# zoj613/OccuSpytial

Measured on AMD Instinct MI355X. Metric: Gibbs iterations/sec on 100x100 ICAR lattice, 4 chains; 1/2/4/8 GPUs, higher is better.
Workload: dtype f64; 1 GPU; 100x100 queen ICAR lattice, 10000 sites, 5 visits/site, p=q=2, 4 chains per GPU batched in every kernel (BASELINE configs[1] data, the metric's 4 chains); chains_per_gpu=4, total_chains=4, sites=10000, visit_rows=50000, parallelism=chains sharded 4/GPU, no data-path collective; one GPU, communicator=single process, problem_transport=none, krylov_cap=0, stalls=0, solve_form=k_iter, one XCD per chain, solve_workgroups_per_chain=23, main_stream_cus=160, fused_fallbacks=0, threads_per_block=64

## Files before the change

### occuspytial_amd/csrc/occ_kernels.hpp

```cpp
#pragma once
#include <float.h>
#include <hip/hip_runtime.h>
#include <stdint.h>

#include "occ_plan.hpp"
#include "occ_rng.hpp"
#include "occ_state.hpp"

namespace occ {


#ifndef OCC_SLOT_ALIGN
#define OCC_SLOT_ALIGN 8
#endif
struct alignas(OCC_SLOT_ALIGN) Slot {
    double beta1, beta, oldb, alfa, dbar, epsln, phibar, rhs1, rhs2, tnorm2, gmax, gmin, cs, sn, root;
    double ibeta;
    int itn;
    int istop;
    int done;
    int pad;
};

#define OCC_SLOT_FIELDS(X) \
// ... 279 lines not shown

__device__ __forceinline__ void reduce_partials_lds(const double *part, int nq, int nw, double *lds_out)
{
    const int lane = threadIdx.x & 63, wave = threadIdx.x >> 6, nwb = blockDim.x >> 6;
    for (int qi = wave; qi < nq; qi += nwb) {
        double s = 0.0;
        const double *pq = part + (size_t)qi * nw;
        for (int b0 = lane; b0 < nw; b0 += 512) {
            double v[8];
#pragma unroll
            for (int r = 0; r < 8; ++r) {
                const int b = b0 + 64 * r;
                const double t = pq[min(b, nw - 1)];
                v[r] = (b < nw) ? t : 0.0;
            }
#pragma unroll
            for (int r = 0; r < 8; ++r) s += v[r];
        }
        s = wave_sum(s);
        if (lane == 0) lds_out[qi] = s;
    }
    __syncthreads();
}

struct PartialEmitter {
    double *out;
    int nb, blk, nq;
    __device__ __forceinline__ void emit(int t, double v)
    {
        extern __shared__ double s_gpart[];
        const double r = wave_sum(v);
        if ((threadIdx.x & 63) == 0) {
            if (blockDim.x == 64) out[(size_t)t * nb + blk] = r;
            else s_gpart[(threadIdx.x >> 6) * nq + t] = r;
        }
    }
    __device__ __forceinline__ void finish()
    {
        extern __shared__ double s_gpart[];
        if (blockDim.x == 64) return;
        __syncthreads();
        const int nw = blockDim.x >> 6;
        for (int t = threadIdx.x; t < nq; t += blockDim.x) {
            double acc = 0.0;
            for (int w = 0; w < nw; ++w) acc += s_gpart[w * nq + t];
            out[(size_t)t * nb + blk] = acc;
        }
    }
};
__host__ __device__ constexpr size_t generic_lds_bytes(int nq, int threads) { return threads == 64 ? 0 : sizeof(double) * (size_t)(threads / 64) * nq; }

__device__ __forceinline__ void slice_of(const Ctx &c, int i, int &base, int &width)
{
    const int slice = i >> 6;
    if (c.ell_w > 0) {
        width = c.ell_w;
        base = slice * c.ell_w * 64;
    } else {
        base = c.sell_ptr[slice];
        width = (c.sell_ptr[slice + 1] - base) >> 6;
    }
}




__device__ __forceinline__ double eta_rhs_site(double om, double xb, double z, double en, double up, double sqrt_tau)
{
    const double b = fma(-om, xb, z - 0.5);
    return fma(sqrt_tau, up, fma(sqrt(om), en, b));
}
__device__ __forceinline__ double eta_project(double2 xz, double a) { return fma(a, xz.y, xz.x); }
__device__ __forceinline__ double beta_rhs_term(double om, double eta, double z) { return fma(-om, eta, z - 0.5); }

__device__ inline bool precision_mvnorm_dev(int d, const double *acc ,
                                            const double *prec0, const double *pbm, uint64_t key, uint32_t it,
                                            uint32_t stream, double *U, double *work, double *out, const double *eps_inj = nullptr)
{
    double *r = work, *o = work + d;
    int t = 0;
    for (int a = 0; a < d; ++a)
        for (int b = a; b < d; ++b) U[a * d + b] = acc[t++] + prec0[a * d + b];
    for (int a = 0; a < d; ++a) r[a] = acc[t++] + pbm[a];
    bool ok = true;
    for (int j = 0; j < d; ++j) {
        double s = U[j * d + j];
        for (int k = 0; k < j; ++k) s -= U[k * d + j] * U[k * d + j];
        if (!(s > 0.0)) ok = false;
        const double ujj = sqrt(s);
        U[j * d + j] = ujj;
        for (int i = j + 1; i < d; ++i) {
            double v = U[j * d + i];
            for (int k = 0; k < j; ++k) v -= U[k * d + j] * U[k * d + i];
            U[j * d + i] = v / ujj;
        }
    }
    for (int i = d - 1; i >= 0; --i) {
        o[i] = 0.0;
    }
    for (int k = 0; k < d; ++k) {
        const double e = eps_inj ? eps_inj[k] : block_normal(key, (uint32_t)k, 0, it, stream);
        for (int i = k; i < d; ++i) o[i] += U[k * d + i] * e;
    }
    for (int i = 0; i < d; ++i) o[i] += r[i];
    for (int i = 0; i < d; ++i) {
        double v = o[i];
        for (int k = 0; k < i; ++k) v -= U[k * d + i] * o[k];
        o[i] = v / U[i * d + i];
    }
    for (int i = d - 1; i >= 0; --i) {
        double v = o[i];
        for (int k = i + 1; k < d; ++k) v -= U[i * d + k] * o[k];
        o[i] = v / U[i * d + i];
    }
    for (int i = 0; i < d; ++i) out[i] = o[i];
    return ok;
}

template <int D, class Normal>
__device__ __forceinline__ bool precision_mvnorm_with(const double (&acc)[nacc(D)], const double *prec0, const double *pbm, double (&out)[D],
                                                      Normal normal)
{
    double U[D][D], r[D], o[D];
    int t = 0;
#pragma unroll
    for (int a = 0; a < D; ++a)
#pragma unroll
        for (int b = a; b < D; ++b) U[a][b] = acc[t++] + prec0[a * D + b];
#pragma unroll
    for (int a = 0; a < D; ++a) r[a] = acc[t++] + pbm[a];
    bool ok = true;
#pragma unroll
    for (int j = 0; j < D; ++j) {
        double sj = U[j][j];
#pragma unroll
        for (int k = 0; k < j; ++k) sj -= U[k][j] * U[k][j];
        if (!(sj > 0.0)) ok = false;
        const double ujj = sqrt(sj);
        U[j][j] = ujj;
#pragma unroll
        for (int i = j + 1; i < D; ++i) {
            double v = U[j][i];
#pragma unroll
            for (int k = 0; k < j; ++k) v -= U[k][j] * U[k][i];
            U[j][i] = v / ujj;
        }
    }
#pragma unroll
    for (int i = 0; i < D; ++i) o[i] = 0.0;
#pragma unroll
    for (int k = 0; k < D; ++k) {
        const double e = normal(k);
#pragma unroll
        for (int i = k; i < D; ++i) o[i] += U[k][i] * e;
    }
#pragma unroll
    for (int i = 0; i < D; ++i) o[i] += r[i];
#pragma unroll
    for (int i = 0; i < D; ++i) {
        double v = o[i];
#pragma unroll
        for (int k = 0; k < i; ++k) v -= U[k][i] * o[k];
        o[i] = v / U[i][i];
    }
#pragma unroll
    for (int i = D - 1; i >= 0; --i) {
        double v = o[i];
#pragma unroll
        for (int k = i + 1; k < D; ++k) v -= U[i][k] * o[k];
        o[i] = v / U[i][i];
    }
#pragma unroll
    for (int i = 0; i < D; ++i) out[i] = o[i];
    return ok;
}

template <int D>
__device__ __forceinline__ bool precision_mvnorm_reg(const double (&acc)[nacc(D)], const double *prec0, const double *pbm,
                                                     uint64_t key, uint32_t it, uint32_t stream, double (&out)[D],
                                                     const double *eps_inj = nullptr)
{
    return precision_mvnorm_with<D>(acc, prec0, pbm, out,
                                    [=](int k) { return eps_inj ? eps_inj[k] : block_normal(key, (uint32_t)k, 0, it, stream); });
}


enum : int { SYNC_MAIN = 0, SYNC_ALPHA = 16, SYNC_NOISE = 32, SYNC_MAIN_SEQ = 48, SYNC_SIDE_SEQ = 52, SYNC_ABORT = 56, SYNC_DEBUG = 57, SYNC_WORDS = 64 };
constexpr unsigned SYNC_SPIN_LIMIT = 1u << 19;

__device__ __forceinline__ unsigned sync_read(const unsigned *p)
{
    return __hip_atomic_load(p, __ATOMIC_RELAXED, __HIP_MEMORY_SCOPE_AGENT);
}
__device__ __forceinline__ void sync_set(unsigned *p, unsigned v)
{
    __hip_atomic_store(p, v, __ATOMIC_RELAXED, __HIP_MEMORY_SCOPE_AGENT);
}
__device__ __forceinline__ bool sync_wait(unsigned *sync, int word, unsigned target)
{
    unsigned spins = 0;
    while ((int)(sync_read(sync + word) - target) < 0) {
        __builtin_amdgcn_s_sleep(4);
        ++spins;
        if ((spins & 63u) == 0u && sync_read(sync + SYNC_ABORT) != 0u) return false;
        if (spins > SYNC_SPIN_LIMIT) {
            sync_set(sync + SYNC_ABORT, 1u);
            return false;
        }
    }
    return true;
}
__device__ __forceinline__ double load_agent(const double *p)
{
    return __hip_atomic_load(p, __ATOMIC_RELAXED, __HIP_MEMORY_SCOPE_AGENT);
}
__device__ __forceinline__ uint64_t uniform_u64(uint64_t v)
{
    const unsigned lo = (unsigned)__builtin_amdgcn_readfirstlane((int)(unsigned)v), hi = (unsigned)__builtin_amdgcn_readfirstlane((int)(unsigned)(v >> 32));
    return ((uint64_t)hi << 32) | lo;
}
__device__ __forceinline__ double uniform_f64(double v) { return __longlong_as_double((long long)uniform_u64((uint64_t)__double_as_longlong(v))); }

__global__ void __launch_bounds__(64) k_stream_probe_wait(unsigned *w)
{
    if (threadIdx.x != 0) return;
    unsigned seen = 0u, spins = 0u;
    for (; spins < (1u << 13); ++spins) {
        if (sync_read(w) != 0u) { seen = 1u; break; }
        __builtin_amdgcn_s_sleep(16);
    }
    w[16] = seen;
    w[17] = spins;
}
__global__ void __launch_bounds__(64) k_stream_probe_set(unsigned *w)
{
    if (threadIdx.x == 0) sync_set(w, 1u);
}

__global__ void __launch_bounds__(256) k_checksum(const unsigned char *__restrict__ data, unsigned long long bytes, unsigned long long *__restrict__ out)
{
    const unsigned long long nw = (bytes + 7ull) / 8ull;
    unsigned long long acc = 0ull;
    for (unsigned long long i = (unsigned long long)blockIdx.x * blockDim.x + threadIdx.x; i < nw; i += (unsigned long long)gridDim.x * blockDim.x) {
        unsigned long long w = 0ull;
        if (8ull * i + 8ull <= bytes) w = *reinterpret_cast<const unsigned long long *>(data + 8ull * i);
        else
            for (unsigned long long b = 8ull * i; b < bytes; ++b) w |= (unsigned long long)data[b] << (8ull * (b - 8ull * i));
        unsigned long long x = w + 0x9E3779B97F4A7C15ull * (i + 1ull);
        x = (x ^ (x >> 30)) * 0xBF58476D1CE4E5B9ull;
        x = (x ^ (x >> 27)) * 0x94D049BB133111EBull;
        acc += x ^ (x >> 31);
    }
    atomicAdd(out, acc);
}

__global__ void __launch_bounds__(256) k_snapshot(const double *__restrict__ eta, double *__restrict__ s_eta, const uint8_t *__restrict__ z, uint8_t *__restrict__ s_z,
                                                  const double2 *__restrict__ x, double2 *__restrict__ s_x, unsigned long long count,
                                                  const double *__restrict__ theta, double *__restrict__ s_theta, unsigned long long count_theta,
                                                  unsigned long long *__restrict__ clock,
                                                  ChainScalars *__restrict__ scs, int n_chains, int parity, uint32_t n_iter, uint32_t burnin, uint32_t keep)
{
    if (clock != nullptr && blockIdx.x == 0 && threadIdx.x < 4) clock[threadIdx.x] = threadIdx.x == 0 ? ~0ull : 0ull;
    if (scs != nullptr && blockIdx.x == 0) {
        for (int ch = (int)threadIdx.x; ch < n_chains; ch += (int)blockDim.x) {
            ChainScalars &sc = scs[ch];
            Ctl &ctl = sc.ctl[parity];
            sc.it_base = ctl.it;
            sc.it_stop = ctl.it + n_iter;
            sc.burnin = burnin;
            sc.keep = keep;
            ctl.koff = 0;
        }
    }
    for (unsigned long long i = (unsigned long long)blockIdx.x * blockDim.x + threadIdx.x; i < count; i += (unsigned long long)gridDim.x * blockDim.x) {
        s_eta[i] = eta[i];
        s_z[i] = z[i];
        s_x[i] = x[i];
    }
    for (unsigned long long i = (unsigned long long)blockIdx.x * blockDim.x + threadIdx.x; i < count_theta; i += (unsigned long long)gridDim.x * blockDim.x) s_theta[i] = theta[i];
}

__global__ void __launch_bounds__(64) k_gate(const Ctx *__restrict__ cp, ChainScalars *__restrict__ scs)
{
    const Ctx &c = *cp;
    if (c.sync == nullptr || threadIdx.x != 0) return;
    const unsigned j = c.sync[SYNC_SIDE_SEQ];
    if (c.sync[SYNC_DEBUG] != 0u) return;
    sync_set(c.sync + SYNC_NOISE, j);
    if (!sync_wait(c.sync, SYNC_MAIN, j)) scs[0].err = -2;
}

#define OCC_KARGS const Ctx *__restrict__ cp, ChainScalars *__restrict__ scs, Slot *__restrict__ slots, int chain_base, int e

__device__ __forceinline__ double quad_site(const Ctx &c, const double *eta, int i, double eta_i)
{
    const int lane = i & 63;
    int base, width;
    slice_of(c, i, base, width);
    double qe = c.qdiag[i] * eta_i;
    for (int k = 0; k < width; ++k) qe = fma(c.sell_val[base + k * 64 + lane], eta[c.sell_col[base + k * 64 + lane]], qe);
    return eta_i * qe;
}

template <int P>
__device__ __forceinline__ void omega_b_body(const Ctx &c, uint64_t key, const double (&beta)[P], int chain, uint32_t it, int blk,
                                             bool per_wave = false)
{
    const int n = c.n;
    const double *eta = c.eta + (size_t)chain * n;
    double om = 0.0;
    {
        const int i = blk * blockDim.x + threadIdx.x;
        if (i < n) {
            double xb = 0.0;
#pragma unroll
            for (int a = 0; a < P; ++a) xb += c.Xt[(size_t)a * n + i] * beta[a];
            om = pg1_draw(key, (uint32_t)i, it, STREAM_OMEGA_B, xb + eta[i]);
        }
    }
    int t = (int)threadIdx.x;
    asm volatile("" : "+v"(t));
    const int i = blk * (int)blockDim.x + t;
    double quad[1] = {0.0};
    if (i < n) {
        c.omega_b[it & 1][(size_t)chain * n + i] = om;
        quad[0] = quad_site(c, eta, i, eta[i]);
    }
    if (per_wave) {
        const double t = wave_sum(quad[0]);
        const int slice = blk * (int)(blockDim.x >> 6) + (int)(threadIdx.x >> 6);
        if ((threadIdx.x & 63) == 0 && slice < c.nb_n) c.part_quad[(size_t)chain * c.nb_n + slice] = t;
        return;
    }
    block_partials<1>(quad, c.part_quad + (size_t)chain * c.nb_n, c.nb_n, blk);
}

__device__ __forceinline__ void omega_b_body_g(const Ctx &c, const ChainScalars &sc, int chain, uint32_t it, int blk, bool per_wave = false)
{
    const int n = c.n, i = blk * blockDim.x + threadIdx.x;
    double quad[1] = {0.0};
    if (i < n) {
        const size_t ci = (size_t)chain * n + i;
        const double *eta = c.eta + (size_t)chain * n;
        double xb = 0.0;
        for (int a = 0; a < c.p; ++a) xb += c.Xt[(size_t)a * n + i] * sc.beta[a];
        const double eta_i = eta[i];
        c.omega_b[it & 1][ci] = pg1_draw(sc.key, (uint32_t)i, it, STREAM_OMEGA_B, xb + eta_i);
        quad[0] = quad_site(c, eta, i, eta_i);
    }
    if (per_wave) {
        const double t = wave_sum(quad[0]);
        const int slice = blk * (int)(blockDim.x >> 6) + (int)(threadIdx.x >> 6);
        if ((threadIdx.x & 63) == 0 && slice < c.nb_n) c.part_quad[(size_t)chain * c.nb_n + slice] = t;
        return;
    }
    block_partials<1>(quad, c.part_quad + (size_t)chain * c.nb_n, c.nb_n, blk);
}

template <int P>
__global__ void __launch_bounds__(256) k_omega_b(OCC_KARGS)
{
    const Ctx &c = *cp;
    const Tile tile = tile_of_block(chain_base);
    const int chain = tile.chain, blk = tile.blk;
    const ChainScalars &sc = scs[chain];
    const Ctl ctl = sc.ctl[e];
    if (ctl.koff || ctl.it >= sc.it_stop || sc.err != 0) return;
    if constexpr (P == 0) {
        omega_b_body_g(c, sc, chain, ctl.it, blk);
    } else {
        double beta[P];
#pragma unroll
        for (int a = 0; a < P; ++a) beta[a] = sc.beta[a];
        omega_b_body<P>(c, sc.key, beta, chain, ctl.it, blk);
    }
}

__global__ void __launch_bounds__(256) k_quad(OCC_KARGS)
{
    const Ctx &c = *cp;
    const Tile tile = tile_of_block(chain_base);
    const int chain = tile.chain, blk = tile.blk;
    const int n = c.n, i = blk * blockDim.x + threadIdx.x;
    const double *eta = c.eta + (size_t)chain * n;
    double quad[1] = {0.0};
    if (i < n) quad[0] = quad_site(c, eta, i, eta[i]);
    block_partials<1>(quad, c.part_quad + (size_t)chain * c.nb_n, c.nb_n, blk);
}

__device__ __forceinline__ void noise_site(const Ctx &c, uint64_t key, int chain, int i, uint32_t it)
{
    const int n = c.n, lane = i & 63;
    int base, width;
    slice_of(c, i, base, width);
    if (c.dense_F != nullptr) width = 0;
    double u = 0.0;
    for (int k = 0; k < width; ++k) {
        const int j = c.sell_col[base + k * 64 + lane];
        const double w = -c.sell_val[base + k * 64 + lane];
        if (w > 0.0) {
            const uint32_t lo = (uint32_t)min(i, j), hi = (uint32_t)max(i, j);
            const double t = sqrt(w) * block_normal(key, lo, hi, it, STREAM_ETA_EDGE);
            u += (i < j) ? t : -t;
        }
    }
    const size_t ci = (size_t)chain * n + i;
    if (c.dense_F == nullptr) c.uprior[it & 1][ci] = u;
    else if (i < c.dense_m) c.dense_eps[it & 1][(size_t)chain * c.dense_m + i] = block_normal(key, (uint32_t)i, 0, it, STREAM_ETA_DENSE);
    c.enorm[it & 1][ci] = block_normal(key, (uint32_t)i, 0, it, STREAM_ETA_SITE);
}

template <int NCH>
__global__ void __launch_bounds__(256) k_prior_dense(const Ctx *__restrict__ cp, ChainScalars *__restrict__ scs, int chain0, int e, int ahead)
{
    const Ctx &c = *cp;
    const int row = blockIdx.x * 4 + (int)(threadIdx.x >> 6), lane = threadIdx.x & 63;
    if (row >= c.n) return;
    const int m = c.dense_m;
    uint32_t it[NCH];
    bool on[NCH];
    bool any = false;
#pragma unroll
    for (int q = 0; q < NCH; ++q) {
        const int ch = chain0 + q;
        on[q] = false;
        it[q] = 0;
        if (ch < c.C) {
            const ChainScalars &sc = scs[ch];
            const Ctl ctl = sc.ctl[e];
            on[q] = !(ctl.koff || ctl.it >= sc.it_stop || sc.err != 0);
            it[q] = ctl.it + (uint32_t)ahead;
        }
        any = any || on[q];
    }
    if (!any) return;
    const double *F = c.dense_F + (size_t)row * m;
    double acc[NCH];
#pragma unroll
    for (int q = 0; q < NCH; ++q) acc[q] = 0.0;
    for (int j = lane; j < m; j += 64) {
        const double f = F[j];
#pragma unroll
        for (int q = 0; q < NCH; ++q)
            if (on[q]) acc[q] = fma(f, c.dense_eps[it[q] & 1][(size_t)(chain0 + q) * m + j], acc[q]);
    }
#pragma unroll
    for (int q = 0; q < NCH; ++q) {
        const double t = wave_sum(acc[q]);
        if (on[q] && lane == 0) c.uprior[it[q] & 1][(size_t)(chain0 + q) * c.n + row] = t;
    }
}

__global__ void __launch_bounds__(256) k_noise(OCC_KARGS, int ahead, int sync_on)
{
    __shared__ double s_red[NACC_G], s_U[MAXG * MAXG], s_work[2 * MAXG], s_alpha[MAXG];
    const Ctx &c = *cp;
    const Tile tile = tile_of_block_shared(c, 2, (c.n + (int)blockDim.x - 1) / (int)blockDim.x, chain_base);
    const int chain = tile.chain, blk = tile.blk;
    const bool synced = sync_on && c.sync;
    if (synced && blockIdx.x == 0 && blockIdx.y == 0 && threadIdx.x == 0) {
        const unsigned j = c.sync[SYNC_SIDE_SEQ];
        c.sync[SYNC_SIDE_SEQ] = j + 1u;
    }
    if (chain < 0) return;
    ChainScalars &sc = scs[chain];
    const Ctl ctl = sc.ctl[e];
    const bool idle = ctl.koff || ctl.it >= sc.it_stop || sc.err != 0;
    if (ahead == 1 && blk == 0) {
        if (!idle) {
            const int Q = c.q;
            reduce_partials_lds(c.part_alpha + (size_t)chain * nacc(Q) * c.nb_r, nacc(Q), c.nb_r, s_red);
            if (threadIdx.x == 0) {
                const double *a_prec = c.hyp, *a_pbm = c.hyp + Q * Q;
                const bool ok = precision_mvnorm_dev(Q, s_red, a_prec, a_pbm, sc.key, ctl.it, STREAM_ALPHA, s_U, s_work, s_alpha, nullptr);
                if (!ok) sc.err = -4;
                for (int a = 0; a < Q; ++a) __hip_atomic_store(&sc.alpha[a], s_alpha[a], __ATOMIC_RELAXED, __HIP_MEMORY_SCOPE_AGENT);
            }
        }
        if (synced && threadIdx.x == 0) {
            asm volatile("s_waitcnt vmcnt(0)" ::: "memory");
            __hip_atomic_fetch_add(c.sync + SYNC_ALPHA, 1u, __ATOMIC_RELAXED, __HIP_MEMORY_SCOPE_AGENT);
        }
    }
    if (idle) return;
    const uint32_t it_for = ctl.it + (uint32_t)ahead;
    if (blk == 0 && threadIdx.x == 0) {
        Cursor g(sc.key, 0u, it_for, STREAM_TAU);
        sc.tau_gamma[it_for & 1] = std_gamma(g, c.tau_shape);
    }
    if (blk == 0 && threadIdx.x >= 64 && (int)threadIdx.x - 64 < c.p) {
        const uint32_t k = threadIdx.x - 64u;
        sc.beta_eps[it_for & 1][k] = block_normal(sc.key, k, 0, it_for, STREAM_BETA);
    }
    const int i = blk * blockDim.x + threadIdx.x;
    if (i >= c.n) return;
    noise_site(c, sc.key, chain, i, it_for);
}

template <int INJ>
__global__ void __launch_bounds__(256) k_eta_init(OCC_KARGS)
{
    __builtin_amdgcn_s_setprio(3);
    const Ctx &c = *cp;
    const Tile tile = tile_of_block(chain_base);
    const int chain = tile.chain, blk = tile.blk;
    ChainScalars &sc = scs[chain];
    const Ctl ctl = sc.ctl[e];
    if (ctl.koff || ctl.it >= sc.it_stop || sc.err != 0) return;
    const int n = c.n, i = blk * blockDim.x + threadIdx.x;
    const uint32_t it = ctl.it;
    double quad[1];
    reduce_partials<1>(c.part_quad + (size_t)chain * c.nb_n, c.nb_n, quad);
    const double rate = 0.5 * quad[0] + c.tau_rate;
    double tau;
    if (INJ) {
        tau = c.inj->tau_from_gamma ? (1.0 / rate) * c.inj->gamma : sc.tau;
    } else {
        tau = (1.0 / rate) * sc.tau_gamma[it & 1];
    }
    if (blk == 0 && threadIdx.x == 0) {
        sc.tau = tau;
        Slot s = {};
        slot_store(&slots[(size_t)chain * NSLOT], s);
    }
    const double st = sqrt(tau);
    if (i < n) {
        const size_t ci = (size_t)chain * n + i;
        const double2 *X0 = c.Xv + (size_t)chain * n;
        const double om = c.omega_b[it & 1][ci];
        const double xb = xdot(c.Xt, n, i, sc.beta, c.p);
        const double y = eta_rhs_site(om, xb, (double)c.z[ci], c.enorm[it & 1][ci], c.uprior[it & 1][ci], st);
        c.rhs[ci] = y;
        const double2 x0 = X0[i];
        const double d = tau * c.qdiag[i] + om;
        double ax = d * x0.x, az = d * x0.y;
        const int lane = i & 63;
        int base, width;
        slice_of(c, i, base, width);
        for (int k = 0; k < width; ++k) {
            const int j = c.sell_col[base + k * 64 + lane];
            const double a = tau * c.sell_val[base + k * 64 + lane];
            const double2 xj = X0[j];
            ax = fma(a, xj.x, ax);
            az = fma(a, xj.y, az);
        }
        double2 r;
        r.x = y - ax;
        r.y = 1.0 - az;
        c.Pv[0][ci] = r;
    }
}

template <class A>
__device__ __forceinline__ void projection_partials(const A &c, int chain, int i, int blk)
{
    double v[2] = {0.0, 0.0};
    if (i < c.n) {
        const double2 x = c.Xv[(size_t)chain * c.n + i];
        v[0] = x.x;
        v[1] = x.y;
    }
    block_partials<2>(v, c.part_proj + (size_t)chain * 2 * c.nb_n, c.nb_n, blk);
}

#ifndef OCC_STAMP
#define OCC_STAMP(n)
#endif


struct KryStep {
    double ca, cb, cc;
    double sj, oldeps, delta, denom, phi;
    bool rotate;
    bool stop;
};

struct KryPre {
    double Anorm, rn2, b1sq;
    bool root_tiny, root_small, ill_cond, no_norm;
    double t_ab, delta, gbar, gbar2, sj;
};
__device__ __forceinline__ double rsqrt_nr(double x)
{
    double y = __builtin_amdgcn_rsq(x);
#pragma unroll
    for (int it = 0; it < 2; ++it) {
        const double h = 0.5 * y;
        const double err = fma(-(x * y), h, 0.5);
        y = fma(y, err, y);
    }
    return y;
}

__device__ __forceinline__ void minres_pre_a(const Slot &s, KryPre &q)
{
    const double eps = DBL_EPSILON, rtol = 1e-5;
    const double tn2 = s.tnorm2, root2 = s.root, tiny2 = 0x1p-106, rtol2 = rtol * rtol;
    q.Anorm = tn2;
    q.no_norm = tn2 == 0.0;
    q.root_tiny = !q.no_norm && root2 <= tiny2 * tn2;
    q.root_small = !q.no_norm && root2 <= rtol2 * tn2;
    q.ill_cond = s.gmax >= (0.1 / eps) * s.gmin;
    q.rn2 = s.phibar * s.phibar;
    q.b1sq = s.beta1 * s.beta1;
}
__device__ __forceinline__ void minres_pre_c(const Slot &s, KryPre &q)
{
    q.t_ab = fma(s.beta, s.beta, s.alfa * s.alfa);
    q.delta = fma(s.sn, s.alfa, s.cs * s.dbar);
    q.gbar = fma(-s.cs, s.alfa, s.sn * s.dbar);
    q.gbar2 = q.gbar * q.gbar;
    q.sj = s.ibeta;
}
__device__ __forceinline__ KryPre minres_pre(const Slot &s)
{
    KryPre q;
    minres_pre_a(s, q);
    minres_pre_c(s, q);
    return q;
}
__device__ __forceinline__ bool minres_post_a(Slot &s, const KryPre &q, int k, double xn2, long long maxiter)
{
    if (k < 4) return false;
    const double eps = DBL_EPSILON, rtol = 1e-5;
    const int j = k - 3;
// ... 698 lines not shown
        double acc[nacc(Q)];
        omega_a_row<Q, INJ>(c, sc, chain, ctl.it, blk * blockDim.x + threadIdx.x, acc);
        block_partials<nacc(Q)>(acc, c.part_alpha + (size_t)chain * nacc(Q) * c.nb_r, c.nb_r, blk);
    }
}

template <int INJ>
__global__ void __launch_bounds__(512) k_alpha_draw(OCC_KARGS, int sync_on)
{
    __shared__ double s_red[NACC_G], s_U[MAXG * MAXG], s_work[2 * MAXG];
    const Ctx &c = *cp;
    const int chain = chain_base + blockIdx.x;
    ChainScalars &sc = scs[chain];
    const Ctl ctl = sc.ctl[e];
    if (!(ctl.koff || ctl.it >= sc.it_stop || sc.err != 0)) {
        const int Q = c.q;
        reduce_partials_lds(c.part_alpha + (size_t)chain * nacc(Q) * c.nb_r, nacc(Q), c.nb_r, s_red);
        if (threadIdx.x == 0) {
            const double *a_prec = c.hyp, *a_pbm = c.hyp + Q * Q;
            const bool ok = precision_mvnorm_dev(Q, s_red, a_prec, a_pbm, sc.key, ctl.it, STREAM_ALPHA, s_U, s_work, sc.alpha,
                                                 INJ ? c.inj->alpha_eps : nullptr);
            if (!ok) sc.err = -4;
        }
    }
    (void)sync_on;
}

enum : int { SITE_PSI = 0, SITE_OCC = 1, SITE_Z = 2, SITE_ETA = 3, SITE_ETA2 = 4, SITE_NACC = 5 };
__device__ __forceinline__ void site_add(const Ctx &c, int chain, int i, double psi, double occ, double z, double eta)
{
    const size_t Cn = (size_t)c.C * c.n;
    double *a = c.site_acc + (size_t)chain * c.n + i;
    a[SITE_PSI * Cn] += psi;
    a[SITE_OCC * Cn] += occ;
    a[SITE_Z * Cn] += z;
    a[SITE_ETA * Cn] += eta;
    a[SITE_ETA2 * Cn] = fma(eta, eta, a[SITE_ETA2 * Cn]);
}

enum : int { LL_LIK = 0, LL_LOG = 1, LL_LOG2 = 2, LL_NACC = 3 };
__device__ __forceinline__ void ll_add(const Ctx &c, int chain, int i, double lik, double ll)
{
    const size_t Cn = (size_t)c.C * c.n;
    double *a = c.ll_acc + (size_t)chain * c.n + i;
    a[LL_LIK * Cn] += lik;
    a[LL_LOG * Cn] += ll;
    a[LL_LOG2 * Cn] = fma(ll, ll, a[LL_LOG2 * Cn]);
}
__device__ __forceinline__ double lsig_e(double a, double e) { return fmin(a, 0.0) - log1p(e); }
__device__ __forceinline__ double expit_e(double a, double e) { return a < 0.0 ? e / (1.0 + e) : 1.0 / (1.0 + e); }

template <int INJ, class XB, class WA>
__device__ __forceinline__ int z_update_site_ll(const Ctx &c, uint64_t key, int chain, int i, uint32_t it, double eta_i, bool stats_on,
                                                 XB xb_of, WA wa_of)
{
    const int sidx = c.site_sidx[i], n = c.n;
    const bool not_surveyed = sidx < 0;
    const bool seen = !not_surveyed && c.obs_site[sidx];
    const double a0 = xb_of() + eta_i, e0 = exp(-fabs(a0));
    const double num1 = expit_e(a0, e0);
    double pr = num1;
    if (!not_surveyed) {
        double prod = 1.0, ll = seen ? lsig_e(a0, e0) : 0.0;
        const int r0 = c.site_ptr[sidx], r1 = c.site_ptr[sidx + 1];
        for (int r = r0; r < r1; ++r) {
            const double wa = wa_of(r), e = exp(-fabs(wa));
            if (seen) {
                ll += lsig_e(c.yrow[r] ? -wa : wa, e);
            } else {
                const double ex = expit_e(wa, e);
                prod = (r == r0) ? ex : prod * ex;
            }
        }
        if (seen) {
            if (stats_on) site_add(c, chain, i, num1, 1.0, 1.0, eta_i);
            ll_add(c, chain, i, exp(ll), ll);
            return 1;
        }
        const double num = num1 * prod;
        const double den = (1.0 - num1) + num;
        pr = num / den;
        ll_add(c, chain, i, den, log(den));
    }
    const double u = INJ ? c.inj->z_u[i] : block_uniform(key, (uint32_t)i, 0, it, STREAM_Z);
    c.z[(size_t)chain * n + i] = (u < pr) ? 1 : 0;
    if (stats_on) site_add(c, chain, i, num1, pr, (u < pr) ? 1.0 : 0.0, eta_i);
    return (u < pr) ? 1 : 0;
}

template <int P, int INJ = 0, int STATS = 0>
__device__ __forceinline__ int z_update_site(const Ctx &c, uint64_t key, int chain, int i, uint32_t it, const double (&beta)[P],
                                              const double (&alpha)[MAXC], double eta_i, bool stats_on = false, bool ll_on = false)
{
    if constexpr (STATS >= 2) {
        if (ll_on) {
            return z_update_site_ll<INJ>(
                c, key, chain, i, it, eta_i, stats_on,
                [&]() {
                    double xb = 0.0;
#pragma unroll
                    for (int a = 0; a < P; ++a) xb = fma(c.Xt[(size_t)a * c.n + i], beta[a], xb);
                    return xb;
                },
                [&](int r) {
                    double wa = 0.0;
#pragma unroll
                    for (int a = 0; a < MAXC; ++a)
                        if (a < c.q) wa = fma(c.Wt[(size_t)a * c.R + r], -alpha[a], wa);
                    return wa;
                });
        }
    }
    const int sidx = c.site_sidx[i];
    const bool not_surveyed = sidx < 0;
    if (!not_surveyed && c.obs_site[sidx]) {
        if constexpr (STATS) {
            if (stats_on) {
                double xb = 0.0;
#pragma unroll
                for (int a = 0; a < P; ++a) xb = fma(c.Xt[(size_t)a * c.n + i], beta[a], xb);
                site_add(c, chain, i, expit(xb + eta_i), 1.0, 1.0, eta_i);
            }
        }
        return 1;
    }
    const int n = c.n, Q = c.q;
    double xb = 0.0;
#pragma unroll
    for (int a = 0; a < P; ++a) xb = fma(c.Xt[(size_t)a * n + i], beta[a], xb);
    const double num1 = expit(xb + eta_i);
    double pr = num1;
    if (!not_surveyed) {
        double prod = 1.0;
        const int r0 = c.site_ptr[sidx], r1 = c.site_ptr[sidx + 1];
        for (int r = r0; r < r1; ++r) {
            double wa = 0.0;
#pragma unroll
            for (int a = 0; a < MAXC; ++a)
                if (a < Q) wa = fma(c.Wt[(size_t)a * c.R + r], -alpha[a], wa);
            const double ex = expit(wa);
            prod = (r == r0) ? ex : prod * ex;
        }
        const double num = num1 * prod;
        pr = num / ((1.0 - num1) + num);
    }
    const double u = INJ ? c.inj->z_u[i] : block_uniform(key, (uint32_t)i, 0, it, STREAM_Z);
    c.z[(size_t)chain * n + i] = (u < pr) ? 1 : 0;
    if constexpr (STATS) {
        if (stats_on) site_add(c, chain, i, num1, pr, (u < pr) ? 1.0 : 0.0, eta_i);
    }
    return (u < pr) ? 1 : 0;
}
template <int P>
__device__ __forceinline__ void record_draws(const Ctx &c, const ChainScalars &sc, int chain, uint32_t it, const double (&alpha)[MAXC],
                                             const double (&beta)[P], double tau)
{
    const uint32_t rel = it - sc.it_base;
    if (c.rec == nullptr || rel < sc.burnin || rel - sc.burnin >= sc.keep) return;
    const int Q = c.q;
    double *row = c.rec + ((size_t)chain * sc.keep + (rel - sc.burnin)) * (size_t)(Q + P + 1);
#pragma unroll
    for (int a = 0; a < MAXC; ++a)
        if (a < Q) row[a] = alpha[a];
#pragma unroll
    for (int a = 0; a < P; ++a) row[Q + a] = beta[a];
    row[Q + P] = tau;
}

constexpr int REGION_MAX = 256;
__device__ __forceinline__ void region_count(uint32_t *__restrict__ row, int G, int g, int zi)
{
    __shared__ unsigned s_occ[REGION_MAX];
    const bool one = zi != 0 && g >= 0;
    for (int k = threadIdx.x; k < G; k += blockDim.x) s_occ[k] = 0u;
    __syncthreads();
    if (G == 1) {
        const unsigned long long m = __ballot(one);
        if ((threadIdx.x & 63u) == 0u && m != 0ull) atomicAdd(&s_occ[0], (unsigned)__popcll(m));
    } else if (one) {
        atomicAdd(&s_occ[g], 1u);
    }
    __syncthreads();
    for (int k = threadIdx.x; k < G; k += blockDim.x) {
        const unsigned v = s_occ[k];
        if (v != 0u) atomicAdd(row + k, v);
    }
}
__device__ __forceinline__ uint32_t *region_row(const Ctx &c, const ChainScalars &sc, int chain, uint32_t it)
{
    const uint32_t rel = it - sc.it_base;
    if (!(sc.site_on & OUT_REGION) || c.occ_rec == nullptr || rel < sc.burnin || rel - sc.burnin >= sc.keep) return nullptr;
    return c.occ_rec + ((size_t)chain * sc.keep + (rel - sc.burnin)) * (size_t)c.region_G;
}

enum : int { PPC_T_OBS = 0, PPC_T_REP = 1, PPC_DET_REP = 2, PPC_SITES_REP = 3, PPC_NCOL = 4 };
__device__ __forceinline__ unsigned long long ppc_fx(double x) { return __double2ull_rn(x * 0x1.0p32); }

__device__ __forceinline__ void ppc_count(unsigned long long *__restrict__ row, const unsigned long long (&term)[PPC_NCOL])
{
    __shared__ unsigned long long s_ppc[PPC_NCOL];
    if (threadIdx.x < PPC_NCOL) s_ppc[threadIdx.x] = 0ull;
    __syncthreads();
    unsigned long long w[PPC_NCOL];
#pragma unroll
    for (int k = 0; k < PPC_NCOL; ++k) w[k] = wave_sum_u64(term[k]);
    if ((threadIdx.x & 63u) == 0u) {
#pragma unroll
        for (int k = 0; k < PPC_NCOL; ++k)
            if (w[k] != 0ull) atomicAdd(&s_ppc[k], w[k]);
    }
    __syncthreads();
    if (threadIdx.x < PPC_NCOL) {
        const unsigned long long v = s_ppc[threadIdx.x];
        if (v != 0ull) atomicAdd(row + threadIdx.x, v);
    }
}
__device__ __forceinline__ unsigned long long *ppc_row(const Ctx &c, const ChainScalars &sc, int chain, uint32_t it)
{
    const uint32_t rel = it - sc.it_base;
    if (!(sc.site_on & OUT_PPC) || c.ppc_rec == nullptr || rel < sc.burnin || rel - sc.burnin >= sc.keep) return nullptr;
    return c.ppc_rec + ((size_t)chain * sc.keep + (rel - sc.burnin)) * (size_t)PPC_NCOL;
}
template <class XB, class WA>
__device__ __forceinline__ int z_update_site_ppc(const Ctx &c, uint64_t key, int chain, int i, uint32_t it, double eta_i, bool stats_on,
                                                 bool ll_on, XB xb_of, WA wa_of, unsigned long long (&term)[PPC_NCOL])
{
    const int sidx = c.site_sidx[i], n = c.n;
    const bool not_surveyed = sidx < 0;
    const bool seen = !not_surveyed && c.obs_site[sidx];
    const double a0 = xb_of() + eta_i, e0 = exp(-fabs(a0));
    const double num1 = expit_e(a0, e0);
    double pr = num1, E = 0.0;
    int y_obs = 0, y_rep = 0, zi = 1;
    if (!not_surveyed) {
        double prod = 1.0, ll = seen ? lsig_e(a0, e0) : 0.0;
        const int r0 = c.site_ptr[sidx], r1 = c.site_ptr[sidx + 1];
        for (int r = r0; r < r1; ++r) {
            const double wa = wa_of(r), e = exp(-fabs(wa));
            const double d = expit_e(-wa, e);
            const double ur = block_uniform(key, (uint32_t)r, 0, it, STREAM_PPC);
            E += d;
            y_rep += (ur < d) ? 1 : 0;
            if (seen) {
                const int y = c.yrow[r] ? 1 : 0;
                y_obs += y;
                if (ll_on) ll += lsig_e(y ? -wa : wa, e);
            } else {
                const double ex = expit_e(wa, e);
                prod = (r == r0) ? ex : prod * ex;
            }
        }
        if (seen) {
            if (stats_on) site_add(c, chain, i, num1, 1.0, 1.0, eta_i);
            if (ll_on) ll_add(c, chain, i, exp(ll), ll);
        } else {
            const double num = num1 * prod;
            const double den = (1.0 - num1) + num;
            pr = num / den;
            if (ll_on) ll_add(c, chain, i, den, log(den));
        }
    }
    if (!seen) {
        const double u = block_uniform(key, (uint32_t)i, 0, it, STREAM_Z);
        zi = (u < pr) ? 1 : 0;
        c.z[(size_t)chain * n + i] = (uint8_t)zi;
        if (stats_on) site_add(c, chain, i, num1, pr, zi ? 1.0 : 0.0, eta_i);
    }
    if (!not_surveyed && zi) {
        const double se = sqrt(E), da = sqrt((double)y_obs) - se, db = sqrt((double)y_rep) - se;
        term[PPC_T_OBS] = ppc_fx(da * da);
        term[PPC_T_REP] = ppc_fx(db * db);
        term[PPC_DET_REP] = (unsigned long long)y_rep;
        term[PPC_SITES_REP] = y_rep > 0 ? 1ull : 0ull;
    }
    return zi;
}


template <int P, int STATS = 0>
__device__ __forceinline__ void z_ob_body(const Ctx &c, ChainScalars *__restrict__ scs, int chain_base, int e, bool synced, unsigned seq,
                                          bool per_wave, int debug_skip = 0,
                                          bool beta_ready = false)
{
    __shared__ int s_wait_ok, s_beta_ok;
    __shared__ double s_beta[P];
    const Tile tile = tile_of_block_shared(c, 0, 2 * (per_wave ? (c.n + (int)blockDim.x - 1) / (int)blockDim.x : c.nb_n), chain_base);
    const int chain = tile.chain, blk = tile.blk;
    if (chain < 0) return;
    ChainScalars &sc = scs[chain];
    constexpr int NQB = nacc(P);
    const bool draws = per_wave && !beta_ready && threadIdx.x < 64;
    const double *part_b = c.part_beta + (size_t)chain * NQB * c.nb_n;
    constexpr bool SUMS_PRE = P <= 4, EPS_PRE = P <= 2;
    double pre[PartialRounds<NQB>::R][NQB], eps2[2][P];
    if (draws) {
        if constexpr (SUMS_PRE) partials_load<NQB>(part_b, c.nb_n, 0, pre);
        if constexpr (EPS_PRE) {
#pragma unroll
            for (int h = 0; h < 2; ++h)
#pragma unroll
                for (int a = 0; a < P; ++a) eps2[h][a] = load_agent(&sc.beta_eps[h][a]);
        }
    }
    const uint64_t key = uniform_u64(sc.key);
    const Ctl ctl = sc.mid[e];
    const uint32_t it_stop = sc.it_stop;
    const int err0 = sc.err;
    asm volatile("" ::"s"(ctl.it), "s"(ctl.koff), "s"(it_stop), "s"(err0));
    const bool skip = ctl.koff || ctl.it >= it_stop || err0 != 0;
    const int nb = per_wave ? (c.n + (int)blockDim.x - 1) / (int)blockDim.x : c.nb_n;
    const uint32_t it = ctl.it;
    const bool writer = (blk == 0 && threadIdx.x == 0);
    if (writer) {
        Ctl nx = ctl;
        if (!skip) nx.it = it + 1;
        sc.ctl[e ^ 1] = nx;
        if (chain == chain_base && c.iter_clock != nullptr && c.iter_clock[1] != 0ull) {
            c.iter_clock[2] += c.iter_clock[1] - c.iter_clock[0];
            c.iter_clock[3] += 1ull;
            c.iter_clock[0] = ~0ull;
            c.iter_clock[1] = 0ull;
        }
        if (chain == chain_base && synced) c.sync[SYNC_MAIN_SEQ + (e ^ 1)] = seq + 1u;
        if (c.claim != nullptr) {
#pragma unroll
            for (int x = 0; x < 8; ++x) c.claim[(size_t)chain * 16 + x] = 0u;
        }
    }
    if (skip) return;
    double beta[P];
    if (beta_ready) {
#pragma unroll
        for (int a = 0; a < P; ++a) beta[a] = sc.beta[a];
    } else {
        double sums[NQB];
        if (!per_wave || !SUMS_PRE) reduce_partials<NQB>(part_b, c.nb_n, sums);
        else if (draws) {
#pragma unroll
            for (int r = 0; r < PartialRounds<NQB>::R; ++r)
#pragma unroll
                for (int qi = 0; qi < NQB; ++qi) asm volatile("" : "+v"(pre[r][qi]));
            if constexpr (EPS_PRE) {
#pragma unroll
                for (int h = 0; h < 2; ++h)
#pragma unroll
                    for (int a = 0; a < P; ++a) asm volatile("" : "+v"(eps2[h][a]));
            }
            reduce_partials_wave<NQB, true>(part_b, c.nb_n, pre, sums);
        }
        const double *b_prec = c.hyp + c.q * c.q + c.q, *b_pbm = b_prec + P * P;
        bool ok = true;
        if (!per_wave || threadIdx.x < 64) {
            if (EPS_PRE && per_wave) {
                ok = precision_mvnorm_with<P>(sums, b_prec, b_pbm, beta, [&](int k) {
                    const double odd = eps2[1][k], even = eps2[0][k];
                    return (it & 1u) ? odd : even;
                });
            } else {
                const double *eps = sc.beta_eps[it & 1];
                ok = precision_mvnorm_with<P>(sums, b_prec, b_pbm, beta, [=](int k) { return load_agent(eps + k); });
            }
            if (per_wave && threadIdx.x == 0) {
                s_beta_ok = ok ? 1 : 0;
#pragma unroll
                for (int a = 0; a < P; ++a) s_beta[a] = beta[a];
            }
        }
        if (per_wave) {
            __syncthreads();
            ok = s_beta_ok != 0;
#pragma unroll
            for (int a = 0; a < P; ++a) beta[a] = s_beta[a];
        }
        if (writer) {
            if (!ok) sc.err = -4;
#pragma unroll
            for (int a = 0; a < P; ++a) sc.beta[a] = beta[a];
        }
    }
    (void)nb;
#pragma unroll
    for (int a = 0; a < P; ++a) beta[a] = uniform_f64(beta[a]);
    if (blk & 1) {
        if (debug_skip & 2) return;
        omega_b_body<P>(c, key, beta, chain, it + 1u, blk >> 1, per_wave);
        return;
    }
    const int Q = c.q;
    double alpha[MAXC];
    if (synced) {
        if (threadIdx.x == 0) s_wait_ok = sync_wait(c.sync, SYNC_ALPHA, (seq + 1u) * (unsigned)c.C) ? 1 : 0;
        __syncthreads();
        if (!s_wait_ok && writer) sc.err = -2;
#pragma unroll
        for (int a = 0; a < MAXC; ++a) alpha[a] = (a < Q) ? load_agent(&sc.alpha[a]) : 0.0;
    } else {
#pragma unroll
        for (int a = 0; a < MAXC; ++a) alpha[a] = (a < Q) ? sc.alpha[a] : 0.0;
    }
    if (writer) record_draws<P>(c, sc, chain, it, alpha, beta, sc.tau);
    const int n = c.n, i = (blk >> 1) * blockDim.x + threadIdx.x;
    if constexpr (STATS == 4) {
        const uint32_t on = sc.site_on;
        const bool kept = it - sc.it_base >= sc.burnin, stats_on = (on & OUT_SITE) && kept, ll_on = (on & OUT_LL) && kept;
        if (debug_skip & 1) return;
        if (writer && stats_on) c.site_count[chain] += 1.0;
        if (writer && ll_on) c.ll_count[chain] += 1.0;
        uint32_t *row = region_row(c, sc, chain, it);
        unsigned long long *prow = ppc_row(c, sc, chain, it);
        const int g = (row != nullptr && i < n) ? (int)c.region_id[i] : -1;
        int zi = 0;
        unsigned long long term[PPC_NCOL] = {0ull, 0ull, 0ull, 0ull};
        if (i < n) {
            const double eta_i = c.eta[(size_t)chain * n + i];
            if (prow != nullptr) {
                zi = z_update_site_ppc(
                    c, key, chain, i, it, eta_i, stats_on, ll_on,
                    [&]() {
                        double xb = 0.0;
#pragma unroll
                        for (int a = 0; a < P; ++a) xb = fma(c.Xt[(size_t)a * c.n + i], beta[a], xb);
                        return xb;
                    },
                    [&](int r) {
                        double wa = 0.0;
#pragma unroll
                        for (int a = 0; a < MAXC; ++a)
                            if (a < c.q) wa = fma(c.Wt[(size_t)a * c.R + r], -alpha[a], wa);
                        return wa;
                    },
                    term);
            } else {
                zi = z_update_site<P, 0, 3>(c, key, chain, i, it, beta, alpha, eta_i, stats_on, ll_on);
            }
        }
        if (row != nullptr) region_count(row, c.region_G, g, zi);
        if (prow != nullptr) ppc_count(prow, term);
    } else if constexpr (STATS == 3) {
        const uint32_t on = sc.site_on;
        const bool kept = it - sc.it_base >= sc.burnin, stats_on = (on & OUT_SITE) && kept, ll_on = (on & OUT_LL) && kept;
        if (debug_skip & 1) return;
        if (writer && stats_on) c.site_count[chain] += 1.0;
        if (writer && ll_on) c.ll_count[chain] += 1.0;
        uint32_t *row = region_row(c, sc, chain, it);
        const int g = (row != nullptr && i < n) ? (int)c.region_id[i] : -1;
        int zi = 0;
        if (i < n) zi = z_update_site<P, 0, 3>(c, key, chain, i, it, beta, alpha, c.eta[(size_t)chain * n + i], stats_on, ll_on);
        if (row != nullptr) region_count(row, c.region_G, g, zi);
    } else if constexpr (STATS == 2) {
        const uint32_t on = sc.site_on;
        const bool kept = it - sc.it_base >= sc.burnin, stats_on = (on & OUT_SITE) && kept, ll_on = (on & OUT_LL) && kept;
        if (writer && stats_on && !(debug_skip & 1)) c.site_count[chain] += 1.0;
        if (writer && ll_on && !(debug_skip & 1)) c.ll_count[chain] += 1.0;
        if (i >= n || (debug_skip & 1)) return;
        z_update_site<P, 0, 2>(c, key, chain, i, it, beta, alpha, c.eta[(size_t)chain * n + i], stats_on, ll_on);
    } else if constexpr (STATS) {
        const bool stats_on = sc.site_on != 0u && it - sc.it_base >= sc.burnin;
        if (writer && stats_on && !(debug_skip & 1)) c.site_count[chain] += 1.0;
        if (i >= n || (debug_skip & 1)) return;
        z_update_site<P, 0, 1>(c, key, chain, i, it, beta, alpha, c.eta[(size_t)chain * n + i], stats_on);
    } else {
    if (i >= n || (debug_skip & 1)) return;
    z_update_site<P>(c, key, chain, i, it, beta, alpha, c.eta[(size_t)chain * n + i]);
    }
}

template <int INJ, int STATS = 0>
__device__ __forceinline__ int z_update_site_g(const Ctx &c, const ChainScalars &sc, int chain, int i, uint32_t it, double eta_i,
                                                bool stats_on = false, bool ll_on = false)
{
    if constexpr (STATS >= 2) {
        if (ll_on) {
            return z_update_site_ll<INJ>(
                c, sc.key, chain, i, it, eta_i, stats_on,
                [&]() {
                    double xb = 0.0;
                    for (int a = 0; a < c.p; ++a) xb = fma(c.Xt[(size_t)a * c.n + i], sc.beta[a], xb);
                    return xb;
                },
                [&](int r) {
                    double wa = 0.0;
                    for (int a = 0; a < c.q; ++a) wa = fma(c.Wt[(size_t)a * c.R + r], -sc.alpha[a], wa);
                    return wa;
                });
        }
    }
    const int sidx = c.site_sidx[i];
    const bool not_surveyed = sidx < 0;
    if (!not_surveyed && c.obs_site[sidx]) {
        if constexpr (STATS) {
            if (stats_on) {
                double xb = 0.0;
                for (int a = 0; a < c.p; ++a) xb = fma(c.Xt[(size_t)a * c.n + i], sc.beta[a], xb);
                site_add(c, chain, i, expit(xb + eta_i), 1.0, 1.0, eta_i);
            }
        }
        return 1;
    }
    const int n = c.n, P = c.p, Q = c.q;
    double xb = 0.0;
    for (int a = 0; a < P; ++a) xb = fma(c.Xt[(size_t)a * n + i], sc.beta[a], xb);
    const double num1 = expit(xb + eta_i);
    double pr = num1;
    if (!not_surveyed) {
        double prod = 1.0;
        const int r0 = c.site_ptr[sidx], r1 = c.site_ptr[sidx + 1];
        for (int r = r0; r < r1; ++r) {
            double wa = 0.0;
            for (int a = 0; a < Q; ++a) wa = fma(c.Wt[(size_t)a * c.R + r], -sc.alpha[a], wa);
            const double ex = expit(wa);
            prod = (r == r0) ? ex : prod * ex;
        }
        const double num = num1 * prod;
        pr = num / ((1.0 - num1) + num);
    }
    const double u = INJ ? c.inj->z_u[i] : block_uniform(sc.key, (uint32_t)i, 0, it, STREAM_Z);
    c.z[(size_t)chain * n + i] = (u < pr) ? 1 : 0;
    if constexpr (STATS) {
        if (stats_on) site_add(c, chain, i, num1, pr, (u < pr) ? 1.0 : 0.0, eta_i);
    }
    return (u < pr) ? 1 : 0;
}

template <int STATS = 0>
__device__ __forceinline__ void z_ob_body_g(const Ctx &c, ChainScalars *__restrict__ scs, int chain_base, int e, bool per_wave, int debug_skip)
{
    const Tile tile = tile_of_block(chain_base);
    const int chain = tile.chain, blk = tile.blk;
    ChainScalars &sc = scs[chain];
    const Ctl ctl = sc.mid[e];
    const bool skip = ctl.koff || ctl.it >= sc.it_stop || sc.err != 0;
    const uint32_t it = ctl.it;
    const bool writer = (blk == 0 && threadIdx.x == 0);
    if (writer) {
        Ctl nx = ctl;
        if (!skip) nx.it = it + 1;
        sc.ctl[e ^ 1] = nx;
    }
    if (skip) return;
    if (blk & 1) {
        if (debug_skip & 2) return;
        omega_b_body_g(c, sc, chain, it + 1u, blk >> 1, per_wave);
        return;
    }
    if (writer) {
        const uint32_t rel = it - sc.it_base;
        if (c.rec != nullptr && rel >= sc.burnin && rel - sc.burnin < sc.keep) {
            double *row = c.rec + ((size_t)chain * sc.keep + (rel - sc.burnin)) * (size_t)(c.q + c.p + 1);
            for (int a = 0; a < c.q; ++a) row[a] = sc.alpha[a];
            for (int a = 0; a < c.p; ++a) row[c.q + a] = sc.beta[a];
            row[c.q + c.p] = sc.tau;
        }
    }
    const int n = c.n, i = (blk >> 1) * blockDim.x + threadIdx.x;
    if constexpr (STATS == 4) {
        const uint32_t on = sc.site_on;
        const bool kept = it - sc.it_base >= sc.burnin, stats_on = (on & OUT_SITE) && kept, ll_on = (on & OUT_LL) && kept;
        if (debug_skip & 1) return;
        if (writer && stats_on) c.site_count[chain] += 1.0;
        if (writer && ll_on) c.ll_count[chain] += 1.0;
        uint32_t *row = region_row(c, sc, chain, it);
        unsigned long long *prow = ppc_row(c, sc, chain, it);
        const int g = (row != nullptr && i < n) ? (int)c.region_id[i] : -1;
        int zi = 0;
        unsigned long long term[PPC_NCOL] = {0ull, 0ull, 0ull, 0ull};
        if (i < n) {
            const double eta_i = c.eta[(size_t)chain * n + i];
            if (prow != nullptr) {
                zi = z_update_site_ppc(
                    c, uniform_u64(sc.key), chain, i, it, eta_i, stats_on, ll_on,
                    [&]() {
                        double xb = 0.0;
                        for (int a = 0; a < c.p; ++a) xb = fma(c.Xt[(size_t)a * c.n + i], sc.beta[a], xb);
                        return xb;
                    },
                    [&](int r) {
                        double wa = 0.0;
                        for (int a = 0; a < c.q; ++a) wa = fma(c.Wt[(size_t)a * c.R + r], -sc.alpha[a], wa);
                        return wa;
                    },
                    term);
            } else {
                zi = z_update_site_g<0, 3>(c, sc, chain, i, it, eta_i, stats_on, ll_on);
            }
        }
        if (row != nullptr) region_count(row, c.region_G, g, zi);
        if (prow != nullptr) ppc_count(prow, term);
    } else if constexpr (STATS == 3) {
        const uint32_t on = sc.site_on;
        const bool kept = it - sc.it_base >= sc.burnin, stats_on = (on & OUT_SITE) && kept, ll_on = (on & OUT_LL) && kept;
        if (debug_skip & 1) return;
        if (writer && stats_on) c.site_count[chain] += 1.0;
        if (writer && ll_on) c.ll_count[chain] += 1.0;
        uint32_t *row = region_row(c, sc, chain, it);
        const int g = (row != nullptr && i < n) ? (int)c.region_id[i] : -1;
        int zi = 0;
        if (i < n) zi = z_update_site_g<0, 3>(c, sc, chain, i, it, c.eta[(size_t)chain * n + i], stats_on, ll_on);
        if (row != nullptr) region_count(row, c.region_G, g, zi);
    } else if constexpr (STATS == 2) {
        const uint32_t on = sc.site_on;
        const bool kept = it - sc.it_base >= sc.burnin, stats_on = (on & OUT_SITE) && kept, ll_on = (on & OUT_LL) && kept;
        if (writer && stats_on && !(debug_skip & 1)) c.site_count[chain] += 1.0;
        if (writer && ll_on && !(debug_skip & 1)) c.ll_count[chain] += 1.0;
        if (i >= n || (debug_skip & 1)) return;
        z_update_site_g<0, 2>(c, sc, chain, i, it, c.eta[(size_t)chain * n + i], stats_on, ll_on);
    } else if constexpr (STATS) {
        const bool stats_on = sc.site_on != 0u && it - sc.it_base >= sc.burnin;
        if (writer && stats_on && !(debug_skip & 1)) c.site_count[chain] += 1.0;
        if (i >= n || (debug_skip & 1)) return;
        z_update_site_g<0, 1>(c, sc, chain, i, it, c.eta[(size_t)chain * n + i], stats_on);
    } else {
    if (i >= n || (debug_skip & 1)) return;
    z_update_site_g<0>(c, sc, chain, i, it, c.eta[(size_t)chain * n + i]);
    }
}

template <int P, int INJ = 0>
__global__ void __launch_bounds__(256) k_beta_draw(OCC_KARGS)
{
    const Ctx &c = *cp;
    const int chain = chain_base + blockIdx.x;
    ChainScalars &sc = scs[chain];
    const Ctl ctl = INJ ? sc.ctl[e] : sc.mid[e];
    if (ctl.koff || ctl.it >= sc.it_stop || sc.err != 0) return;
    if constexpr (P == 0) {
        __shared__ double s_red[NACC_G], s_U[MAXG * MAXG], s_work[2 * MAXG];
        const int p = c.p;
        reduce_partials_lds(c.part_beta + (size_t)chain * nacc(p) * c.nb_n, nacc(p), c.nb_n, s_red);
        if (threadIdx.x == 0) {
            const double *b_prec = c.hyp + c.q * c.q + c.q, *b_pbm = b_prec + p * p;
            const bool ok = precision_mvnorm_dev(p, s_red, b_prec, b_pbm, sc.key, ctl.it, STREAM_BETA, s_U, s_work, sc.beta,
                                                 INJ ? c.inj->beta_eps : sc.beta_eps[ctl.it & 1]);
            if (!ok) sc.err = -4;
        }
        return;
    } else {
    double sums[nacc(P)], beta[P];
    reduce_partials<nacc(P)>(c.part_beta + (size_t)chain * nacc(P) * c.nb_n, c.nb_n, sums);
    const double *b_prec = c.hyp + c.q * c.q + c.q, *b_pbm = b_prec + P * P;
    const bool ok = precision_mvnorm_reg<P>(sums, b_prec, b_pbm, sc.key, ctl.it, STREAM_BETA, beta, INJ ? c.inj->beta_eps : sc.beta_eps[ctl.it & 1]);
    if (threadIdx.x == 0) {
        if (!ok) sc.err = -4;
#pragma unroll
        for (int a = 0; a < P; ++a) sc.beta[a] = beta[a];
    }
    }
}

template <int P>
__global__ void __launch_bounds__(256, 3) k_z_ob(OCC_KARGS, int flags)
{
    __builtin_amdgcn_s_setprio(3);
    const Ctx &c = *cp;
    if constexpr (P == 0) {
        z_ob_body_g(c, scs, chain_base, e, (flags & 2) != 0, (flags >> 3) & 3);
    } else {
        const bool synced = (flags & 1) && c.sync != nullptr;
        const unsigned seq = synced ? (unsigned)__builtin_amdgcn_readfirstlane((int)c.sync[SYNC_MAIN]) : 0u;
        z_ob_body<P>(c, scs, chain_base, e, synced, seq, (flags & 2) != 0, (flags >> 3) & 3, (flags & 4) != 0);
    }
}

template <int P>
__global__ void __launch_bounds__(256, 3) k_z_ob_stats(OCC_KARGS, int flags)
{
    __builtin_amdgcn_s_setprio(3);
    const Ctx &c = *cp;
    if constexpr (P == 0) {
        z_ob_body_g<1>(c, scs, chain_base, e, (flags & 2) != 0, (flags >> 3) & 3);
    } else {
        const bool synced = (flags & 1) && c.sync != nullptr;
        const unsigned seq = synced ? (unsigned)__builtin_amdgcn_readfirstlane((int)c.sync[SYNC_MAIN]) : 0u;
        z_ob_body<P, 1>(c, scs, chain_base, e, synced, seq, (flags & 2) != 0, (flags >> 3) & 3, (flags & 4) != 0);
    }
}

template <int P>
__global__ void __launch_bounds__(256, 3) k_z_ob_ll(OCC_KARGS, int flags)
{
    __builtin_amdgcn_s_setprio(3);
    const Ctx &c = *cp;
    if constexpr (P == 0) {
        z_ob_body_g<2>(c, scs, chain_base, e, (flags & 2) != 0, (flags >> 3) & 3);
    } else {
        const bool synced = (flags & 1) && c.sync != nullptr;
        const unsigned seq = synced ? (unsigned)__builtin_amdgcn_readfirstlane((int)c.sync[SYNC_MAIN]) : 0u;
        z_ob_body<P, 2>(c, scs, chain_base, e, synced, seq, (flags & 2) != 0, (flags >> 3) & 3, (flags & 4) != 0);
    }
}

template <int P>
__global__ void __launch_bounds__(256, 3) k_z_ob_occ(OCC_KARGS, int flags)
{
    __builtin_amdgcn_s_setprio(3);
    const Ctx &c = *cp;
    if constexpr (P == 0) {
        z_ob_body_g<3>(c, scs, chain_base, e, (flags & 2) != 0, (flags >> 3) & 3);
    } else {
        const bool synced = (flags & 1) && c.sync != nullptr;
        const unsigned seq = synced ? (unsigned)__builtin_amdgcn_readfirstlane((int)c.sync[SYNC_MAIN]) : 0u;
        z_ob_body<P, 3>(c, scs, chain_base, e, synced, seq, (flags & 2) != 0, (flags >> 3) & 3, (flags & 4) != 0);
    }
}

// ... 88 lines not shown
```

Baseline: 83480 iterations/s.

## Prefetch eta, X rows and SELL quad-form gathers before beta reduction

```diff
diff --git a/occuspytial_amd/csrc/occ_kernels.hpp b/occuspytial_amd/csrc/occ_kernels.hpp
--- a/occuspytial_amd/csrc/occ_kernels.hpp
+++ b/occuspytial_amd/csrc/occ_kernels.hpp
@@ -605,9 +605,48 @@
     return eta_i * qe;
 }
 
-template <int P>
+struct QuadPre {
+    static constexpr int QW = 8;
+    int base, width, col[QW];
+    double qd, eta_i, val[QW], ev[QW];
+    __device__ __forceinline__ void rows(const Ctx &c, const __attribute__((address_space(1))) double *g_eta, int i)
+    {
+        const int lane = i & 63;
+        slice_of(c, i, base, width);
+        qd = ((const __attribute__((address_space(1))) double *)c.qdiag)[i];
+        eta_i = g_eta[i];
+        if (width > 0) {
+#pragma unroll
+            for (int k = 0; k < QW; ++k) {
+                const int s = base + min(k, width - 1) * 64 + lane;
+                col[k] = ((const __attribute__((address_space(1))) int *)c.sell_col)[s];
+                val[k] = ((const __attribute__((address_space(1))) double *)c.sell_val)[s];
+            }
+        }
+    }
+    __device__ __forceinline__ void gather(const __attribute__((address_space(1))) double *g_eta)
+    {
+        if (width > 0) {
+#pragma unroll
+            for (int k = 0; k < QW; ++k) ev[k] = g_eta[col[k]];
+        }
+    }
+    __device__ __forceinline__ double finish(const Ctx &c, const double *eta, int i) const
+    {
+        const int lane = i & 63;
+        double qe = qd * eta_i;
+        if (width > 0) {
+#pragma unroll
+            for (int k = 0; k < QW; ++k) qe = (k < width) ? fma(val[k], ev[k], qe) : qe;
+        }
+        for (int k = QW; k < width; ++k) qe = fma(c.sell_val[base + k * 64 + lane], eta[c.sell_col[base + k * 64 + lane]], qe);
+        return eta_i * qe;
+    }
+};
+
+template <int P, bool PRE = false>
 __device__ __forceinline__ void omega_b_body(const Ctx &c, uint64_t key, const double (&beta)[P], int chain, uint32_t it, int blk,
-                                             bool per_wave = false)
+                                             bool per_wave = false, const double *x_pre = nullptr, double eta_pre = 0.0)
 {
     const int n = c.n;
     const double *eta = c.eta + (size_t)chain * n;
@@ -616,14 +655,24 @@
         const int i = blk * blockDim.x + threadIdx.x;
         if (i < n) {
             double xb = 0.0;
-#pragma unroll
-            for (int a = 0; a < P; ++a) xb += c.Xt[(size_t)a * n + i] * beta[a];
-            om = pg1_draw(key, (uint32_t)i, it, STREAM_OMEGA_B, xb + eta[i]);
+            if constexpr (PRE) {
+#pragma unroll
+                for (int a = 0; a < P; ++a) xb += x_pre[a] * beta[a];
+                om = pg1_draw(key, (uint32_t)i, it, STREAM_OMEGA_B, xb + eta_pre);
+            } else {
+#pragma unroll
+                for (int a = 0; a < P; ++a) xb += c.Xt[(size_t)a * n + i] * beta[a];
+                om = pg1_draw(key, (uint32_t)i, it, STREAM_OMEGA_B, xb + eta[i]);
+            }
         }
     }
     int t = (int)threadIdx.x;
     asm volatile("" : "+v"(t));
     const int i = blk * (int)blockDim.x + t;
+    if constexpr (PRE) {
+        if (i < n) c.omega_b[it & 1][(size_t)chain * n + i] = om;
+        return;
+    }
     double quad[1] = {0.0};
     if (i < n) {
         c.omega_b[it & 1][(size_t)chain * n + i] = om;
@@ -1928,12 +1977,33 @@
                 for (int a = 0; a < P; ++a) eps2[h][a] = load_agent(&sc.beta_eps[h][a]);
         }
     }
+    const int n = c.n, site = (blk >> 1) * (int)blockDim.x + (int)threadIdx.x;
+    const __attribute__((address_space(1))) double *g_eta = (const __attribute__((address_space(1))) double *)(c.eta + (size_t)chain * n);
+    double x_pre[P], eta_pre = 0.0;
+    QuadPre qp;
+    qp.width = 0;
+#pragma unroll
+    for (int a = 0; a < P; ++a) x_pre[a] = 0.0;
+    constexpr bool ROW_PRE = P <= 7;
+    if (site < n) {
+        if (blk & 1) {
+            if constexpr (ROW_PRE) {
+                const __attribute__((address_space(1))) double *g_X = (const __attribute__((address_space(1))) double *)c.Xt;
+#pragma unroll
+                for (int a = 0; a < P; ++a) x_pre[a] = g_X[(size_t)a * n + site];
+            }
+            eta_pre = g_eta[site];
+        } else {
+            qp.rows(c, g_eta, site);
+        }
+    }
     const uint64_t key = uniform_u64(sc.key);
     const Ctl ctl = sc.mid[e];
     const uint32_t it_stop = sc.it_stop;
     const int err0 = sc.err;
     asm volatile("" ::"s"(ctl.it), "s"(ctl.koff), "s"(it_stop), "s"(err0));
     const bool skip = ctl.koff || ctl.it >= it_stop || err0 != 0;
+    if (!(blk & 1) && site < n) qp.gather(g_eta);
     const int nb = per_wave ? (c.n + (int)blockDim.x - 1) / (int)blockDim.x : c.nb_n;
     const uint32_t it = ctl.it;
     const bool writer = (blk == 0 && threadIdx.x == 0);
@@ -1954,6 +2024,21 @@
         }
     }
     if (skip) return;
+    constexpr bool QUAD_LATE = P <= 3;
+    const auto store_quad = [&]() {
+        double quad[1] = {0.0};
+        if (site < n) quad[0] = qp.finish(c, c.eta + (size_t)chain * n, site);
+        if (per_wave) {
+            const double t = wave_sum(quad[0]);
+            const int slice = (blk >> 1) * (int)(blockDim.x >> 6) + (int)(threadIdx.x >> 6);
+            if ((threadIdx.x & 63) == 0 && slice < c.nb_n) c.part_quad[(size_t)chain * c.nb_n + slice] = t;
+        } else {
+            block_partials<1>(quad, c.part_quad + (size_t)chain * c.nb_n, c.nb_n, blk >> 1);
+        }
+    };
+    if constexpr (!QUAD_LATE) {
+        if (!(blk & 1)) store_quad();
+    }
     double beta[P];
     if (beta_ready) {
 #pragma unroll
@@ -2009,9 +2094,19 @@
     for (int a = 0; a < P; ++a) beta[a] = uniform_f64(beta[a]);
     if (blk & 1) {
         if (debug_skip & 2) return;
-        omega_b_body<P>(c, key, beta, chain, it + 1u, blk >> 1, per_wave);
+        if constexpr (!ROW_PRE) {
+            if (site < n) {
+#pragma unroll
+                for (int a = 0; a < P; ++a) x_pre[a] = c.Xt[(size_t)a * n + site];
+            }
+        }
+#pragma unroll
+        for (int a = 0; a < P; ++a) asm volatile("" : "+v"(x_pre[a]));
+        asm volatile("" : "+v"(eta_pre));
+        omega_b_body<P, true>(c, key, beta, chain, it + 1u, blk >> 1, per_wave, x_pre, eta_pre);
         return;
     }
+    if constexpr (QUAD_LATE) store_quad();
     const int Q = c.q;
     double alpha[MAXC];
     if (synced) {
@@ -2025,7 +2120,7 @@
         for (int a = 0; a < MAXC; ++a) alpha[a] = (a < Q) ? sc.alpha[a] : 0.0;
     }
     if (writer) record_draws<P>(c, sc, chain, it, alpha, beta, sc.tau);
-    const int n = c.n, i = (blk >> 1) * blockDim.x + threadIdx.x;
+    const int i = site;
     if constexpr (STATS == 4) {
         const uint32_t on = sc.site_on;
         const bool kept = it - sc.it_base >= sc.burnin, stats_on = (on & OUT_SITE) && kept, ll_on = (on & OUT_LL) && kept;
```

After: 83710 iterations/s, median of 2. No clear change (+0.3%).
